# JeffWang987/MVSTER

Measured on AMD Instinct MI355X. Metric: depth-maps/sec (DTU 512×640, 5-view, 4-stage) at 1/2/4/8 MI355X, higher is better.
Workload: dtype f32; 1 GPU; DTU mid 512x640, 5 views, 4-stage cascade 8/8/4/4 hyp, B=1 eval, 1 depth map(s) per step per GPU; launch=hipGraph replay, parallelism=replicas x1, depth_maps_in_flight_per_gpu=2

## Files before the change

### include/mvster_hip.h

```cpp
#ifndef MVSTER_HIP_H
#define MVSTER_HIP_H

#ifdef __cplusplus
extern "C" {
#endif

#define MVSTER_OK 0
#define MVSTER_ERR_NULL (-1)
#define MVSTER_ERR_SHAPE (-2)
#define MVSTER_ERR_UNSUPPORTED (-3)
#define MVSTER_ERR_LAUNCH (-4)

int mvster_relative_projection(const float* proj_matrices, float* rt, int B, int N, void* stream);

int mvster_relative_projection_multi(const float* const* proj_matrices, int nstage, float* rt, int B, int N,
                                     void* stream);

int mvster_pack_images(const float* const* imgs, int N, float* out, int B, int H, int W, void* stream);

int mvster_pack_images_u8(const unsigned char* imgs, float* out, int V, int H, int W, void* stream);

int mvster_load_pack_images_u8(const unsigned char* buf, long buf_bytes, const int* desc_host, const int* desc, const void* tables,
                               long table_words, float* out, unsigned char* out_u8, int V, int Hd, int Wd, void* stream);

// ... 36 lines not shown
                                long* origin_ints);

int mvster_warp_agg_bwd_sorted_scratch(int B, int NV, int C, int D, int h, int w, int Hs, int Ws, long* rec_floats, long* ints);
int mvster_warp_agg_bwd_sorted(const float* ref_feat, const float* src_feat, const float* rt, const float* hypo,
                               const float* out, const float* wsum, const float* grad_out, float* grad_ref, float* grad_src,
                               float* rec, int* ints, int B, int NV, int C, int G, int D, int h, int w, int Hs, int Ws,
                               long ref_batch_stride, long src_view_stride, long src_batch_stride, int group_cor,
                               int attn_fuse_d, float attn_temp, void* stream);

int mvster_init_range(const float* depth_values, int ndv, float* out, int B, int D, int h, int w, int inverse,
                      void* stream);

int mvster_schedule_inverse_range(const float* inv_min, const float* inv_max, float* out, int B, int D, int h,
                                  int w, void* stream);

int mvster_schedule_range(const float* cur_depth, const float* interval, float* out, int B, int D, int h, int w,
                          void* stream);

int mvster_select_depth(const float* logits, const float* feat, const float* prob_w, const float* prob_b, int CF,
                        const float* hypo, float* attn, float* depth, float* conf, float* inv_min, float* inv_max,
                        float* logits_out, int B, int D, int h, int w, float split_itv, void* stream);

int mvster_select_depth_bwd(const float* attn, const float* gattn, const float* feat, const float* prob_w, float* dfeat,
                            float* partial, int B, int D, int h, int w, int CF, void* stream);

int mvster_upsample_bilinear(const float* in, float* out, int B, int hi, int wi, int ho, int wo, void* stream);

int mvster_upsample_bilinear_multi(const float* const* ins, float* const* outs, const int* his, const int* wis, int n, int B,
                                   int ho, int wo, void* stream);

int mvster_conv_mfma(const float* in, const float* wpk, const float* scale, const float* shift, const float* skip,
                     const float* zeros, const float* prob_w, const float* prob_b, float* out, const int* geom,
                     int ngeom, const long* woff, int cin, int mt, int nt, int variant, void* stream);

int mvster_conv_small(const float* in, const float* w, const float* scale, const float* shift, const float* skip,
                      float* out, int NB, int H, int W, int cin, int relu, void* stream);

int mvster_conv_narrow(const float* in, const float* w, const float* scale, const float* shift, const float* skip,
                       float* out, int NB, int H, int W, int cin, int relu, int mt, int wpc, void* stream);

int mvster_conv_narrow4(const float* in, const float* w, const float* scale, const float* shift, float* out, int NB, int H,
                        int W, int relu, int mt, int wpc, void* stream);

int mvster_conv_narrow_pair(const float* in, const float* w1, const float* scale1, const float* shift1, const float* w2,
                            const float* scale2, const float* shift2, float* out, int NB, int H, int W, int relu1, int relu2,
                            int wpc, void* stream);

int mvster_conv_narrow_pair_planes(const float* const* imgs, int N, int B, int H, int W, const float* w1, const float* scale1,
                                   const float* shift1, const float* w2, const float* scale2, const float* shift2, float* out,
                                   int relu1, int relu2, int wpc, const float* const* proj_matrices, int nstage, float* rt,
                                   const float* depth_values, int ndv, float* hypo, int D, int h, int w, int inverse,
                                   void* stream);

int mvster_deconv_small(const float* in, const float* w, const float* scale, const float* shift, const float* skip,
                        const float* prob_w, const float* prob_b, float* out, int NB, int Hi, int Wi, int cin,
                        int cout, int relu, void* stream);

int mvster_deconv_select(const float* in, const float* w, const float* scale, const float* shift, const float* skip,
                         const float* prob_w, const float* prob_b, const float* hypo, float* attn, float* depth, float* conf,
                         float* inv_min, float* inv_max, float* logits_out, int B, int D, int Hi, int Wi, int cin, int relu,
                         float split_itv, void* stream);

int mvster_deconv_select_riders(const float* in, const float* w, const float* scale, const float* shift, const float* skip,
                                const float* prob_w, const float* prob_b, const float* hypo, float* attn, float* depth,
                                float* conf, float* inv_min, float* inv_max, float* logits_out, int B, int D, int Hi, int Wi,
                                int cin, int relu, float split_itv, const float* const* up_ins, float* const* up_outs,
// ... 199 lines not shown
```

### mvster_amd/_lib.py

```python
import ctypes
import os

_HERE = os.path.dirname(os.path.abspath(__file__))
LIB_PATH = os.environ.get("MVSTER_LIB") or os.path.join(_HERE, "csrc", "libmvster_hip.so")

ERR_NULL, ERR_SHAPE, ERR_UNSUPPORTED, ERR_LAUNCH = -1, -2, -3, -4
ERRORS = {-1: "NULL pointer", -2: "bad shape", -3: "unsupported channel/tile combination", -4: "kernel launch failed"}

_f = ctypes.c_void_p
_i = ctypes.c_int
_l = ctypes.c_long
_fl = ctypes.c_float

SIGNATURES = {
    "mvster_relative_projection": [_f, _f, _i, _i, _f],
    "mvster_relative_projection_multi": [_f, _i, _f, _i, _i, _f],
    "mvster_pack_images": [_f, _i, _f, _i, _i, _i, _f],
    "mvster_pack_images_u8": [_f, _f, _i, _i, _i, _f],
    "mvster_load_pack_images_u8": [_f, _l, _f, _f, _f, _l, _f, _f, _i, _i, _i, _f],
    "mvster_forward_prologue": [_f, _i, _f, _i, _i, _i, _f, _i, _f, _f, _i, _f, _i, _i, _i, _i, _f],
    "mvster_warp_agg_fwd": [_f, _f, _f, _f, _f, _f] + [_i] * 9 + [_l] * 3 + [_i, _i, _fl, _i, _f],
    "mvster_warp_agg_fwd_indexed": [_f, _f, _f, _f, _f, _f] + [_i] * 10 + [_fl, _i, _f],
    "mvster_warp_agg_fwd_counted": [_f, _f, _f, _f, _f, _f] + [_i] * 9 + [_l] * 3 + [_i, _i, _fl, _i, _f, _f],
    "mvster_warp_agg_fwd_indexed_counted": [_f, _f, _f, _f, _f, _f] + [_i] * 10 + [_fl, _i, _f, _f],
    "mvster_gather_views": [_f, _f, _f, _i, _i, _i, _l, _f],
    "mvster_warp_agg_fwd_sched": [_f] * 6 + [_i, _f, _f, _f] + [_i] * 9 + [_l] * 3 + [_i, _fl, _i, _f],
    "mvster_warp_agg_bwd": [_f] * 11 + [_i] * 9 + [_l] * 3 + [_i, _i, _fl, _f],
    "mvster_warp_agg_bwd_scratch": [_i] * 8 + [_f, _f],
    "mvster_warp_agg_bwd_sorted_scratch": [_i] * 8 + [_f, _f],
    "mvster_warp_agg_bwd_sorted": [_f] * 11 + [_i] * 9 + [_l] * 3 + [_i, _i, _fl, _f],
    "mvster_init_range": [_f, _i, _f, _i, _i, _i, _i, _i, _f],
    "mvster_schedule_inverse_range": [_f, _f, _f, _i, _i, _i, _i, _f],
    "mvster_schedule_range": [_f, _f, _f, _i, _i, _i, _i, _f],
    "mvster_select_depth": [_f, _f, _f, _f, _i, _f, _f, _f, _f, _f, _f, _f, _i, _i, _i, _i, _fl, _f],
    "mvster_select_depth_bwd": [_f, _f, _f, _f, _f, _f, _i, _i, _i, _i, _i, _f],
    "mvster_upsample_bilinear": [_f, _f, _i, _i, _i, _i, _i, _f],
    "mvster_upsample_bilinear_multi": [_f, _f, _f, _f, _i, _i, _i, _i, _f],
    "mvster_conv_mfma": [_f, _f, _f, _f, _f, _f, _f, _f, _f, _f, _i, _f, _i, _i, _i, _i, _f],
    "mvster_conv_small": [_f, _f, _f, _f, _f, _f, _i, _i, _i, _i, _i, _f],
    "mvster_conv_narrow": [_f, _f, _f, _f, _f, _f, _i, _i, _i, _i, _i, _i, _i, _f],
    "mvster_conv_narrow4": [_f, _f, _f, _f, _f, _i, _i, _i, _i, _i, _i, _f],
    "mvster_conv_narrow_pair": [_f, _f, _f, _f, _f, _f, _f, _f, _i, _i, _i, _i, _i, _i, _f],
    "mvster_conv_narrow_pair_planes": [_f] + [_i] * 4 + [_f] * 7 + [_i] * 3 + [_f, _i, _f, _f, _i, _f] + [_i] * 4 + [_f],
    "mvster_deconv_select": [_f] * 14 + [_i] * 6 + [_fl, _f],
    "mvster_deconv_select_riders": [_f] * 14 + [_i] * 6 + [_fl] + [_f] * 4 + [_i] * 3 + [_f],
    "mvster_deconv_small": [_f, _f, _f, _f, _f, _f, _f, _f, _i, _i, _i, _i, _i, _i, _f],
    "mvster_fpn_tail_gather": [_f, _f, _f, _f, _i, _i, _i, _i, _f],
    "mvster_fpn_lateral_up": [_f, _f, _f, _f, _f, _i, _i, _i, _i, _i, _f],
    "mvster_fpn_tail_fused": [_f, _f, _f, _f, _f, _f, _i, _i, _i, _i, _f],
    "mvster_fpn_tail_gather_bwd": [_f, _f, _i, _i, _i, _i, _i, _f],
    "mvster_pack_conv_weights": [_f, _f] + [_i] * 6 + [_l] * 5 + [_i, _f],
    "mvster_pack_wino_weights": [_f, _f, _i, _i, _i, _i, _l, _l, _l, _l, _l, _i, _f],
    "mvster_pack_wino_batch": [_f, _i, _i, _f],
    "mvster_pack_conv_weights_classes": [_f, _f, _i, _i, _i, _i, _i, _f, _f, _f, _f],
    "mvster_conv_wgrad": [_f, _f, _f] + [_i] * 20 + [_f],
    "mvster_conv_wgrad_slots": [_i] * 12,
    "mvster_bn_relu_fwd": [_f, _f, _f, _f, _f, _l, _i, _i, _i, _f],
    "mvster_conv_wgrad_finish": [_f, _f] + [_i] * 10 + [_f],
    "mvster_bn_slots": [_l, _i, _i],
    "mvster_col_sum": [_f, _f, _f, _f, _l, _i, _f],
    "mvster_bn_train_slots": [_l, _i, _i],
    "mvster_bn_train_fwd": [_f] * 10 + [_l, _i, _i, _i, _fl, _fl, _f],
    "mvster_bn_train_bwd": [_f] * 7 + [_l, _i, _i, _i, _f],
    "mvster_conv_wgrad_finish_batch": [_f, _i, _f],
    "mvster_bn_relu_bwd_reduce": [_f] * 11 + [_l, _i, _i, _i, _f],
    "mvster_bn_relu_bwd_apply": [_f] * 8 + [_l, _i, _i, _i, _i, _f],
    "mvster_upsample2x_cl_fwd": [_f, _f, _i, _i, _i, _i, _f],
    "mvster_upsample2x_cl_bwd": [_f, _f, _i, _i, _i, _i, _f],
    "mvster_upsample2x_nearest_cl": [_f, _f, _i, _i, _i, _i, _i, _f],
    "mvster_sinkhorn": [_f, _f, _f, _f, _f, _i, _i, _l, _i, _fl, _f],
    "mvster_sinkhorn_continuous": [_f, _f, _f, _f, _f, _f, _i, _i, _l, _i, _fl, _f],
# ... 83 lines not shown
```

### mvster_amd/conv_plan.py

```python
import ctypes

import numpy as np
import torch

from . import _lib, ops

GEOM = ("B", "Di", "Hi", "Wi", "Do", "Ho", "Wo", "DoF", "HoF", "WoF", "sd", "sh", "sw", "cout", "ntile_total", "relu",
        "skip_mode", "osd", "osh", "osw", "nclass")
GEOM_CLASS = ("kd", "kh", "kw", "pd", "ph", "pw", "od", "oh", "ow", "nsteps")

SKIP_NONE, SKIP_ADD, SKIP_UPSAMPLE_ADD = 0, 1, 2


def _pack_gemm(wk):
    K, N = wk.shape
    Kp, Np = (K + 15) // 16 * 16, (N + 15) // 16 * 16
    full = wk.new_zeros(Kp, Np)
    full[:K, :N] = wk
    return full.view(Kp // 16, 4, 4, Np // 16, 16).permute(0, 3, 1, 4, 2).contiguous().view(-1), Kp // 16


def fold_bn(bn, cout, device):
    if bn is None:
        return torch.ones(cout, device=device), torch.zeros(cout, device=device)
# ... 68 lines not shown


FUSE_TAIL = True
FUSE_SELECT = True
LDS_BUDGET = 12 * 256 * 16
FORCE_VARIANT = None
TPERS16_MIN_VOXELS = 40960
FUSE_CONV0 = True
NARROW_PAIR_WPC = 1
NARROW_PAIR_MIN_PIXELS = 512 * 14 * 64
NARROW_MIN_VOXELS = 64 * 256


def _lds_plan(B, Do, Ho, Wo, kernel, stride, ntile_total):
    kd, kh, kw = kernel
    if kw not in (3, 5) or Wo < 24:
        return None
    for mt in (4, 2):
        ty = 2 * mt
        patch = kd * ((ty - 1) * stride[1] + kh) * (31 * stride[2] + kw) * 64
        if patch > LDS_BUDGET or (mt == 4 and Ho < 6):
            continue
        blocks = -(-Wo // 32) * -(-Ho // ty) * Do * B
        nt = max(n for n in (4, 2, 1) if n <= ntile_total and ntile_total % n == 0)
        while nt > 1 and blocks * (ntile_total // nt) < 512:
            nt //= 2
        return mt, nt
    return None


WINO_RING_INSTANCES = {(0, 1, 3), (0, 2, 3), (1, 2, 3), (2, 2, 3), (0, 4, 3), (1, 4, 3), (2, 4, 3),
                       (0, 4, 1), (1, 4, 1), (2, 4, 1), (0, 2, 1), (1, 2, 1), (2, 2, 1), (0, 1, 1), (2, 1, 1)}
WINO_INSTANCES = {(1, 1), (2, 1), (2, 2), (1, 2)}


def _wino_plan(layer, B, Do, Ho, Wo):
    tiles = B * Do * -(-Ho // 8) * -(-Wo // 32)
    kd = layer.kernel[0]
    if kd == 1 and layer.cin in (16, 32):
        nt = 2 if layer.ntile_total % 2 == 0 else 1
        if tiles * (layer.ntile_total // nt) >= 192:
            return 8 | (1 << 8), 2, nt
        return None
    nt = 2 if (layer.ntile_total % 2 == 0 and tiles * (layer.ntile_total // 2) >= 224) else 1
    if (1, layer.cin // 16, kd) not in WINO_RING_INSTANCES:
        nt = 1
    if tiles * (layer.ntile_total // nt) >= 160 and (0 if nt == 1 else 1, layer.cin // 16, kd) in WINO_RING_INSTANCES:
        return 9, 2, nt
    return None


def _tiles(M, ntile_total, nclass):
    best = None
    for nt in (5, 4, 3, 2, 1):
        if nt > ntile_total or ntile_total % nt:
            continue
        for mt in (4, 2, 1):
            waves = -(-M // (16 * mt)) * (ntile_total // nt) * nclass
            if waves >= 2048:
                return mt, nt
            if best is None or waves > best[0]:
                best = (waves, mt, nt)
    return best[1], best[2]


class ConvLayer:
# ... 182 lines not shown
            ntaps = np.zeros(len(self.classes), dtype=np.int32)
            taps = np.zeros((len(self.classes), 27), dtype=np.int32)
            for i, c in enumerate(self.classes):
                kzs, kys, kxs = c["taps"]
                flat = [(z * kh + y) * kw + x for z in kzs for y in kys for x in kxs]
                ntaps[i] = len(flat)
                taps[i, :len(flat)] = flat
            tab = self._class_pack = (ntaps, np.ascontiguousarray(self.woff, dtype=np.int64), taps)
        ntaps, woff, taps = tab
        rc = _lib.load().mvster_pack_conv_weights_classes(
            w.data_ptr(), self.wpk.data_ptr(), self.cout, self._cin_raw, self.cin, kd * kh * kw, len(self.classes),
            ntaps.ctypes.data_as(ctypes.c_void_p), woff.ctypes.data_as(ctypes.c_void_p), taps.ctypes.data_as(ctypes.c_void_p),
            ops._stream())
        _lib.check(rc, "pack_conv_weights_classes")
        if self.w_deconv is not None:
            self.w_deconv.copy_(w[:, :, 0].permute(2, 3, 0, 1))

    def repack(self, weight, bias=None):
        w = weight.detach().float()
        if w.dim() == 4:
            w = w.unsqueeze(2)
        self._pack(w)
        if bias is not None:
            self.shift[:self.cout] = bias.detach().float() * self.scale[:self.cout]

    def out_shape(self, B, Di, Hi, Wi):
        kd, kh, kw = self.kernel
        s, p = self.stride, self.padding
        if self.transposed:
            return (B, Di * s[0], Hi * s[1], Wi * s[2])
        return (B, (Di + 2 * p[0] - kd) // s[0] + 1, (Hi + 2 * p[1] - kh) // s[1] + 1, (Wi + 2 * p[2] - kw) // s[2] + 1)

    def _geom(self, B, Di, Hi, Wi, skip_mode):
        key = (B, Di, Hi, Wi, skip_mode)
        g = self._geom_cache.get(key)
        if g is None:
            _, DoF, HoF, WoF = self.out_shape(B, Di, Hi, Wi)
            s = self.stride
            if self.transposed:
                Do, Ho, Wo = Di, Hi, Wi
                sd = sh = sw = 1
                osd, osh, osw = s
            else:
                Do, Ho, Wo = DoF, HoF, WoF
                sd, sh, sw = s
                osd = osh = osw = 1
            vals = dict(B=B, Di=Di, Hi=Hi, Wi=Wi, Do=Do, Ho=Ho, Wo=Wo, DoF=DoF, HoF=HoF, WoF=WoF, sd=sd, sh=sh, sw=sw,
                        cout=self.cout, ntile_total=self.ntile_total, relu=int(self.relu), skip_mode=skip_mode,
                        osd=osd, osh=osh, osw=osw, nclass=len(self.classes))
            arr = [vals[k] for k in GEOM]
            for c in self.classes:
                arr += [c[k] for k in GEOM_CLASS]
            mt, nt = _tiles(B * Do * Ho * Wo, self.ntile_total, len(self.classes))
            variant = 0
            lds = None
            if not self.transposed and self.cin % 16 == 0 and skip_mode in (SKIP_NONE, SKIP_ADD):
                lds = _lds_plan(B, Do, Ho, Wo, self.kernel, self.stride, self.ntile_total)
            if lds is not None and FORCE_VARIANT != 0:
                variant, (mt, nt) = 1, lds
            if variant == 0 and self.cin >= 16 and FORCE_VARIANT is None:
                tiles16 = -(-(B * Do * Ho * Wo) // 16)
                waves = -(-tiles16 // mt) * (self.ntile_total // nt) * len(self.classes)
                if waves < 1024 and min(c["nsteps"] for c in self.classes) >= 8:
                    variant, mt = 2, 1
                    nt = 1
                    for cand in (4, 2):
                        if self.ntile_total % cand == 0 and tiles16 * (self.ntile_total // cand) * len(self.classes) >= 512:
                            nt = cand
                            break
            if (FORCE_VARIANT is None and self.wpk_wino is not None and self.prob is None
                    and skip_mode in (SKIP_NONE, SKIP_ADD)):
                wv = _wino_plan(self, B, Do, Ho, Wo)
                if wv is not None:
                    variant, mt, nt = wv
            tuned = tuned_choice(self, B, Di, Hi, Wi, skip_mode)[0] if FORCE_VARIANT is None else None
            if tuned and (tuned[0] & 0xff) in (8, 9) and (self.wpk_wino is None or self.prob is not None):
                tuned = None
            if tuned:
                variant, mt, nt = tuned
            if self.w_small is not None and skip_mode in (SKIP_NONE, SKIP_ADD) and FORCE_VARIANT in (None, 3, 10):
                if FORCE_VARIANT is not None:
                    variant, mt, nt = FORCE_VARIANT, 0, 0
                elif tuned and tuned[0] in (3, 10):
                    variant, mt, nt = tuned
                else:
                    variant, mt, nt = (10, 0, 0) if B * Do * Ho * Wo >= NARROW_MIN_VOXELS else (3, 0, 0)
                if variant == 10 and not hasattr(_lib.load(), "mvster_conv_narrow"):
                    variant = 3
            if (getattr(self, "w_small4", None) is not None and skip_mode == SKIP_NONE and FORCE_VARIANT is None
                    and self.prob is None and B * Do * Ho * Wo >= NARROW_MIN_VOXELS and hasattr(_lib.load(), "mvster_conv_narrow4")):
                variant, mt, nt = 10, 0, 0
            if self.w_deconv is not None and skip_mode in (SKIP_NONE, SKIP_ADD) and FORCE_VARIANT in (None, 4):
                variant = 4
                if (FORCE_VARIANT is None and self.prob is None and self.cin == 16 and self.cout == 8
                        and B * Di * Hi * Wi >= TPERS16_MIN_VOXELS):
                    variant, mt, nt = 5, 2, 1
            if (FORCE_VARIANT is None and self.transposed and self.kernel == (1, 5, 5) and self.stride == (1, 2, 2)
                    and self.padding == (0, 2, 2) and self.cin in (16, 32) and self.prob is None
                    and skip_mode in (SKIP_NONE, SKIP_ADD) and B * Di * Hi * Wi >= TPERS16_MIN_VOXELS):
                variant, mt, nt = 5, 2, 1
            g = (np.asarray(arr, dtype=np.int32), mt, nt, (B, DoF, HoF, WoF), variant)
            self._geom_cache[key] = g
        return g

    def __call__(self, x, skip=None, skip_mode=SKIP_NONE, tiles=None):
        B, Di, Hi, Wi, C = x.shape
        if C != self.cin or not x.is_contiguous() or x.dtype != torch.float32 or not x.is_cuda:
            raise RuntimeError("conv_mfma: bad input (shape %s, cin %d)" % (tuple(x.shape), self.cin))
        if skip is None:
            skip_mode = SKIP_NONE
        geom, mt, nt, oshape, variant = self._geom(B, Di, Hi, Wi, skip_mode)
        if tiles is not None:
# ... 394 lines not shown
```

### mvster_amd/csrc/conv_mfma.hip

```cpp
#include <stdlib.h>

#include <type_traits>

#include "conv_args.hpp"

namespace {

using namespace mvconv;

typedef unsigned u32x4v __attribute__((ext_vector_type(4)));

#ifdef MVSTER_TIMELINE
__device__ unsigned long long* g_tl = nullptr;
#define MV_TL(k)                                                                                              \
    do {                                                                                                      \
        __builtin_amdgcn_sched_barrier(0);                                                                    \
        if (g_tl && (threadIdx.x & 63) == 0)                                                                  \
            g_tl[((size_t)blockIdx.x * 4 + (threadIdx.x >> 6)) * 8 + (k)] = __builtin_amdgcn_s_memtime();     \
        __builtin_amdgcn_sched_barrier(0);                                                                    \
    } while (0)
#define MV_TL_ID()                                                                                            \
    do {                                                                                                      \
        if (g_tl && (threadIdx.x & 63) == 0) {                                                                \
            g_tl[((size_t)blockIdx.x * 4 + (threadIdx.x >> 6)) * 8 + 6] = __builtin_amdgcn_s_getreg(63492);   \
// ... 34 lines not shown
            for (int j = 0; j < 4; ++j) v[j] += k[j];
        } else if (a.skip_mode == 2) {
            const int hh = a.HoF / 2, wh = a.WoF / 2;
            const mv::Lerp ly = mv::make_lerp(oy, hh, a.HoF), lx = mv::make_lerp(ox, wh, a.WoF);
            const float* sk = a.skip + (long)b * hh * wh * a.cout + n0;
            const f32x4v k00 = *reinterpret_cast<const f32x4v*>(sk + ((long)ly.i0 * wh + lx.i0) * a.cout);
            const f32x4v k01 = *reinterpret_cast<const f32x4v*>(sk + ((long)ly.i0 * wh + lx.i1) * a.cout);
            const f32x4v k10 = *reinterpret_cast<const f32x4v*>(sk + ((long)ly.i1 * wh + lx.i0) * a.cout);
            const f32x4v k11 = *reinterpret_cast<const f32x4v*>(sk + ((long)ly.i1 * wh + lx.i1) * a.cout);
#pragma unroll
            for (int j = 0; j < 4; ++j) v[j] = mv::bilerp(ly, lx, k00[j], k01[j], k10[j], k11[j]) + v[j];
        }
        *reinterpret_cast<f32x4v*>(op) = v;
    } else {
        for (int j = 0; j < 4; ++j) {
            if (n0 + j >= a.cout) break;
            float r = v[j];
            if (a.skip_mode == 1) r += a.skip[opix * a.cout + n0 + j];
            op[j] = r;
        }
    }
}

__device__ __forceinline__ void epilogue_store(const ConvArgs& a, f32x4v v, int n0, long opix, int b, int oy, int ox) {
    epilogue_store(a, v, n0, opix, b, oy, ox, *reinterpret_cast<const f32x4v*>(a.scale + n0),
                   *reinterpret_cast<const f32x4v*>(a.shift + n0));
}

constexpr int conv_min_waves(int mt, int nt) {
    const int t = mt * nt;
    return t <= 2 ? 5 : (t <= 4 ? 4 : (t <= 8 ? 3 : 2));
}

template <int CIN, int MT, int NT, bool SPLITK>
__global__ void __launch_bounds__(256, conv_min_waves(MT, NT)) conv_mfma_kernel(ConvArgs a) {
    static_assert(CIN % 4 == 0 && (CIN >= 16 ? CIN % 16 == 0 : 16 % CIN == 0), "channel packing");
    __shared__ f32x4v red[SPLITK ? 3 * MT * NT * 64 : 1];

    const int cls = blockIdx.z;
    const int KD = a.kd[cls], KH = a.kh[cls], KW = a.kw[cls];
    const int PD = a.pd[cls], PH = a.ph[cls], PW = a.pw[cls];
    const int ntaps = KD * KH * KW;
    const mvtaps::TapDivs tdv = a.tapdiv[cls];
    const int nsteps_all = a.nsteps[cls];
    const bool no_pad = a.all_inside[cls] != 0;
    const bool fit = mvtaps::masks_fit(KD, KH, KW);

    const int lane = threadIdx.x & 63;
    const int wave = __builtin_amdgcn_readfirstlane(threadIdx.x >> 6);
    const int lm = lane & 15;
    const int lq = lane >> 4;
    const unsigned Mtot = (unsigned)(a.B * a.Do * a.Ho * a.Wo);
    const int nt0 = blockIdx.y * NT;
    const unsigned ntiles = (Mtot + 15u) >> 4;
    const unsigned ngroups = SPLITK ? (ntiles + MT - 1) / MT : (ntiles + 4 * MT - 1) / (4 * MT);
    for (unsigned grp0 = blockIdx.x; grp0 < ngroups; grp0 += gridDim.x) {
    const unsigned grp = gridDim.x == ngroups ? xcd_remap(grp0, ngroups) : grp0;
    const unsigned tile0 = SPLITK ? grp * MT : (grp * 4u + wave) * MT;
    if (!SPLITK && tile0 * 16u >= Mtot) break;

    int iz0[MT], iy0[MT], ix0[MT];
    unsigned abase[MT];
    unsigned vmask[MT];
    int opix[MT];
    int oyx[MT];
#pragma unroll
    for (int mt = 0; mt < MT; ++mt) {
        unsigned m = (tile0 + mt) * 16u + lm;
        const bool ok = m < Mtot;
        if (!ok) m = 0;
        unsigned r = fast_div(m, a.Wo, a.div_mul[0], a.div_shr[0]);
        const int x = (int)(m - r * (unsigned)a.Wo);
        unsigned r2 = fast_div(r, a.Ho, a.div_mul[1], a.div_shr[1]);
        const int y = (int)(r - r2 * (unsigned)a.Ho);
        const unsigned b = fast_div(r2, a.Do, a.div_mul[2], a.div_shr[2]);
        const int z = (int)(r2 - b * (unsigned)a.Do);
        iz0[mt] = ok ? z * a.sd - PD : -(1 << 20);
        iy0[mt] = y * a.sh - PH;
        ix0[mt] = x * a.sw - PW;
        const int pin0 = (((int)b * a.Di + (ok ? iz0[mt] : 0)) * a.Hi + iy0[mt]) * a.Wi + ix0[mt];
        abase[mt] = (unsigned)(pin0 * CIN + (CIN >= 16 ? lq * 4 : 0)) * 4u;
        vmask[mt] = fit ? mvtaps::voxel_mask(iz0[mt], iy0[mt], ix0[mt], KD, KH, KW, a.Di, a.Hi, a.Wi) : 0u;
        const int oz = z * a.osd + a.od[cls], oy = y * a.osh + a.oh[cls], ox = x * a.osw + a.ow[cls];
        opix[mt] = ok ? (((int)b * a.DoF + oz) * a.HoF + oy) * a.WoF + ox : -1;
        oyx[mt] = (oy << 16) | ox;
    }

    f32x4v acc[MT][NT];
#pragma unroll
    for (int mt = 0; mt < MT; ++mt)
#pragma unroll
        for (int nt = 0; nt < NT; ++nt) acc[mt][nt] = (f32x4v){0.f, 0.f, 0.f, 0.f};

    const long wstep = (long)a.ntile_total * 1024;
    const __amdgpu_buffer_rsrc_t w_rsrc = __builtin_amdgcn_make_buffer_rsrc(
        const_cast<float*>(a.wpk + a.woff[cls] + (long)nt0 * 256), (short)0,
        (int)((unsigned)nsteps_all * (unsigned)wstep - (unsigned)nt0 * 1024u), 0x00020000);
    const unsigned wlane = (unsigned)lane * 16u;

    const __amdgpu_buffer_rsrc_t in_rsrc =
        __builtin_amdgcn_make_buffer_rsrc(const_cast<float*>(a.in), (short)0, (int)a.in_bytes, 0x00020000);
    const int nsteps = mvtaps::wave_steps(nsteps_all, wave, SPLITK);

    auto uni = [](unsigned v) { return CIN >= 16 ? (unsigned)__builtin_amdgcn_readfirstlane((int)v) : v; };
    auto load_step = [&](auto mode, int si, f32x4v (&A)[MT], f32x4v (&Bv)[NT]) {
        constexpr int MODE = decltype(mode)::value;
        const int s = mvtaps::wave_step(si, wave, SPLITK);
        const int tap = mvtaps::step_tap<CIN>(s, lq);
        const int c = CIN >= 16 ? s * 16 - tap * CIN : mvtaps::step_channel<CIN>(s, lq);
        const bool tap_ok = CIN >= 16 || tap < ntaps;
        const mvtaps::Tap t = mvtaps::tap_decode(tap_ok ? tap : 0, KH, KW, tdv);
        const unsigned uoff = uni((unsigned)(mvtaps::tap_offset(t, a.Hi, a.Wi) * CIN + c) * 4u);
        const unsigned sel = MODE == 1 ? uni(mvtaps::tap_select(t, KD, KH)) : 0u;
#pragma unroll
        for (int mt = 0; mt < MT; ++mt) {
            if constexpr (MODE == 0) {
                A[mt] = __builtin_bit_cast(f32x4v, __builtin_amdgcn_raw_buffer_load_b128(in_rsrc, abase[mt], uoff, 0));
            } else {
                const bool ok = tap_ok && (MODE == 1 ? mvtaps::tap_inside(vmask[mt], sel)
                                                     : mvtaps::tap_inside_cmp(iz0[mt], iy0[mt], ix0[mt], t, a.Di, a.Hi, a.Wi));
                const unsigned off = ok ? abase[mt] + uoff : 0xFFFFFFF0u;
                A[mt] = __builtin_bit_cast(f32x4v, __builtin_amdgcn_raw_buffer_load_b128(in_rsrc, off, 0, 0));
            }
        }
        const unsigned woff = (unsigned)s * (unsigned)wstep;
#pragma unroll
        for (int nt = 0; nt < NT; ++nt)
            Bv[nt] = __builtin_bit_cast(f32x4v, __builtin_amdgcn_raw_buffer_load_b128(w_rsrc, wlane + nt * 1024u, woff, 0));
    };

    auto mma_step = [&](const f32x4v (&A)[MT], const f32x4v (&Bv)[NT]) {
#pragma unroll
        for (int j = 0; j < 4; ++j)
#pragma unroll
            for (int mt = 0; mt < MT; ++mt)
#pragma unroll
                for (int nt = 0; nt < NT; ++nt)
                    acc[mt][nt] = __builtin_amdgcn_mfma_f32_16x16x4f32(Bv[nt][j], A[mt][j], acc[mt][nt], 0, 0, 0);
    };

    auto k_loop = [&](auto mode) {
        f32x4v af[MT], bf[NT], ag[MT], bg[NT];
        if (nsteps <= 0) return;
        const int last = nsteps - 1;
        load_step(mode, 0, af, bf);
        int s = 0;
        for (; s + 2 <= nsteps; s += 2) {
            load_step(mode, s + 1, ag, bg);
            mma_step(af, bf);
            load_step(mode, min(s + 2, last), af, bf);
            mma_step(ag, bg);
        }
        if (s < nsteps) mma_step(af, bf);
    };
    if (!fit) {
        f32x4v af[MT], bf[NT];
        for (int s = 0; s < nsteps; ++s) {
            load_step(std::integral_constant<int, 2>{}, s, af, bf);
            mma_step(af, bf);
        }
    } else if (CIN >= 16 && no_pad) {
        k_loop(std::integral_constant<int, CIN >= 16 ? 0 : 1>{});
    } else {
        k_loop(std::integral_constant<int, 1>{});
    }

    if (SPLITK) {
        if (wave > 0) {
#pragma unroll
            for (int mt = 0; mt < MT; ++mt)
#pragma unroll
                for (int nt = 0; nt < NT; ++nt) red[((wave - 1) * MT * NT + mt * NT + nt) * 64 + lane] = acc[mt][nt];
        }
        __syncthreads();
        if (wave > 0) return;
#pragma unroll
        for (int w = 0; w < 3; ++w)
#pragma unroll
            for (int mt = 0; mt < MT; ++mt)
#pragma unroll
                for (int nt = 0; nt < NT; ++nt) {
                    const f32x4v r = red[(w * MT * NT + mt * NT + nt) * 64 + lane];
#pragma unroll
                    for (int j = 0; j < 4; ++j) acc[mt][nt][j] += r[j];
                }
    }

#pragma unroll
    for (int mt = 0; mt < MT; ++mt) {
        if (opix[mt] < 0) continue;
        const int b = a.skip_mode == 2 ? opix[mt] / (a.DoF * a.HoF * a.WoF) : 0;
#pragma unroll
        for (int nt = 0; nt < NT; ++nt) {
            const int n0 = (nt0 + nt) * 16 + lq * 4;
            if (n0 >= a.cout) continue;
            epilogue_store(a, acc[mt][nt], n0, opix[mt], b, oyx[mt] >> 16, oyx[mt] & 0xffff);
        }
    }
    }
}

template <int CIN, int MT, int NT, bool SPLITK>
int launch(const ConvArgs& a, hipStream_t s) {
    const long Mtot = (long)a.B * a.Do * a.Ho * a.Wo;
    if (Mtot >= (1L << 31) || (long)a.B * a.Di * a.Hi * a.Wi >= (1L << 31)) return MVSTER_ERR_SHAPE;
    const long tiles = (Mtot + 15) / 16;
    const long per_block = SPLITK ? MT : 4 * MT;
    long gx = (tiles + per_block - 1) / per_block;
    dim3 grid((unsigned)gx, a.ntile_total / NT, a.nclass);
    MV_NOTE_KERNEL("conv_mfma_kernel<%d, %d, %d, %s>", CIN, MT, NT, SPLITK ? "true" : "false");
    hipLaunchKernelGGL((conv_mfma_kernel<CIN, MT, NT, SPLITK>), grid, dim3(256), 0, s, a);
    return mv_check_launch();
}

template <int CIN>
int dispatch_tiles(const ConvArgs& a, int MT, int NT, bool splitk, hipStream_t s) {
    if (splitk) {
        if constexpr (CIN >= 16) {
#define MV_S(M_, N_) if (MT == M_ && NT == N_) return launch<CIN, M_, N_, true>(a, s);
            MV_S(1, 1) MV_S(1, 2) MV_S(1, 4) MV_S(2, 1) MV_S(2, 2)
#undef MV_S
        }
        return MVSTER_ERR_UNSUPPORTED;
    }
#define MV_T(M_, N_) if (MT == M_ && NT == N_) return launch<CIN, M_, N_, false>(a, s);
    MV_T(1, 1) MV_T(2, 1) MV_T(4, 1) MV_T(1, 2) MV_T(2, 2) MV_T(4, 2) MV_T(1, 4) MV_T(2, 4) MV_T(4, 4)
    if constexpr (CIN == 64) {
        MV_T(1, 5) MV_T(2, 5) MV_T(4, 5)
        MV_T(1, 3) MV_T(2, 3) MV_T(4, 3) MV_T(1, 9) MV_T(2, 9)
    }
#undef MV_T
    return MVSTER_ERR_UNSUPPORTED;
}

struct LdsDivs {
    unsigned mul[6], shr[6];
};
constexpr int kMaxStage = 12;
__device__ __forceinline__ int patch_plane(int npix) { return ((npix * 2 + 7) & ~7) + 4; }
static const bool g_no_wlds = MV_PROBE_ENV("MVSTER_NO_WLDS") != nullptr;

template <int MT, int NT, int KW, int NG, int WN>
__global__ void __launch_bounds__(256) conv_lds_kernel(ConvArgs a, int tiles_x, int tiles_y, LdsDivs dv) {
    extern __shared__ __attribute__((aligned(16))) float patch_raw[];
    MV_TL(0);
    MV_TL_ID();
    f32x4v* patch_base = reinterpret_cast<f32x4v*>(patch_raw);
    f32x4v* wl = patch_base + NG * 1024 + 32;
    constexpr int TY = 2 * MT;
// ... 251 lines not shown
        if (a.kd[c] * a.kh[c] * a.kw[c] > kMaxTaps || a.nsteps[c] < 1) return MVSTER_ERR_SHAPE;
        if (a.kd[c] < 1 || a.kh[c] < 1 || a.kw[c] < 1) return MVSTER_ERR_SHAPE;
        a.tapdiv[c] = mvtaps::make_tap_divs(a.kh[c], a.kw[c]);
    }
    if (a.B <= 0 || a.Do <= 0 || a.Ho <= 0 || a.Wo <= 0 || a.cout <= 0 || a.ntile_total <= 0) return MVSTER_ERR_SHAPE;
    find_divisor((unsigned)a.Wo, a.div_mul[0], a.div_shr[0]);
    find_divisor((unsigned)a.Ho, a.div_mul[1], a.div_shr[1]);
    find_divisor((unsigned)a.Do, a.div_mul[2], a.div_shr[2]);
    {
        const long in_elems = (long)a.B * a.Di * a.Hi * a.Wi * cin;
        const long out_elems = (long)a.B * a.DoF * a.HoF * a.WoF * a.cout;
        if (in_elems >= (1L << 30) || out_elems >= (1L << 31)) return MVSTER_ERR_SHAPE;
        a.in_bytes = (unsigned)(in_elems * 4);
    }
    for (int c = 0; c < a.nclass; ++c) {
        auto inside = [](int n_out, int s, int p, int k, int extent) {
            return -p >= 0 && (n_out - 1) * s - p + (k - 1) < extent;
        };
        a.all_inside[c] = inside(a.Do, a.sd, a.pd[c], a.kd[c], a.Di) && inside(a.Ho, a.sh, a.ph[c], a.kh[c], a.Hi) &&
                          inside(a.Wo, a.sw, a.pw[c], a.kw[c], a.Wi);
    }
    if (a.skip_mode != 0 && !skip) return MVSTER_ERR_NULL;
    if (a.ntile_total % nt != 0) return MVSTER_ERR_SHAPE;
    hipStream_t s = (hipStream_t)stream;
    a.cin = cin;
    if ((variant & 0xff) == 5) return dispatch_pers(a, mt, nt, variant >> 8, s);
    if ((variant & 0xff) == 6) return dispatch_1x1(a, mt, variant >> 8, s);
    if ((variant & 0xff) == 7) return dispatch_pp(a, mt, nt, s);
    if ((variant & 0xff) == 8) return dispatch_wino(a, nt, variant >> 8, false, s);
    if ((variant & 0xff) == 9) return dispatch_wino(a, nt, variant >> 8, true, s);
    if ((variant & 0xff) == 11) return dispatch_b3(a, mt, variant >> 8, s);
    if (prob_w && (a.cout != 8 || a.skip_mode == 2 || variant == 1)) return MVSTER_ERR_UNSUPPORTED;
    if (variant == 1) return dispatch_lds(a, mt, nt, s);
    if (variant != 0 && variant != 2) return MVSTER_ERR_UNSUPPORTED;
    const bool splitk = variant == 2;
    switch (cin) {
        case 4: return dispatch_tiles<4>(a, mt, nt, splitk, s);
        case 8: return dispatch_tiles<8>(a, mt, nt, splitk, s);
        case 16: return dispatch_tiles<16>(a, mt, nt, splitk, s);
        case 32: return dispatch_tiles<32>(a, mt, nt, splitk, s);
        case 64: return dispatch_tiles<64>(a, mt, nt, splitk, s);
        case 80: return dispatch_tiles<80>(a, mt, nt, splitk, s);
        default: return MVSTER_ERR_UNSUPPORTED;
    }
}

#ifdef MVSTER_TIMELINE
extern "C" int mvster_debug_timeline(void* buf) {
    return hipMemcpyToSymbol(HIP_SYMBOL(g_tl), &buf, sizeof(buf)) == hipSuccess ? MVSTER_OK : MVSTER_ERR_LAUNCH;
}
#endif

extern "C" int mvster_mfma_probe(const float* A, const float* B, float* D, void* stream) {
    if (!A || !B || !D) return MVSTER_ERR_NULL;
    hipLaunchKernelGGL(mfma_probe_kernel, dim3(1), dim3(64), 0, (hipStream_t)stream, A, B, D);
    return mv_check_launch();
}

namespace {
__global__ void __launch_bounds__(256) pack_weights_kernel(const float* __restrict__ w, float* __restrict__ wpk, int nsteps,
                                                           int ntile, int cout, int cin, int cin_pad, int kd, int kh, int kw,
                                                           long s_n, long s_c, long s_z, long s_y, long s_x, int flip) {
    const int idx = blockIdx.x * 256 + threadIdx.x;
    if (idx >= nsteps * ntile * 64) return;
    const int lane = idx & 63, t = (idx >> 6) % ntile, st = (idx >> 6) / ntile;
    const int n = t * 16 + (lane & 15);
    const int ntaps = kd * kh * kw;
    f32x4v out;
#pragma unroll
    for (int j = 0; j < 4; ++j) {
        const int k = st * 16 + (lane >> 4) * 4 + j;
        const int tap = k / cin_pad, ci = k - tap * cin_pad;
        float v = 0.0f;
        if (tap < ntaps && ci < cin && n < cout) {
            int kx = tap % kw, ky = (tap / kw) % kh, kz = tap / (kw * kh);
            if (flip) { kx = kw - 1 - kx; ky = kh - 1 - ky; kz = kd - 1 - kz; }
            v = w[(long)n * s_n + (long)ci * s_c + (long)kz * s_z + (long)ky * s_y + (long)kx * s_x];
// ... 72 lines not shown
```

### mvster_amd/csrc/conv_taps.h

```cpp
#pragma once

#if defined(__HIPCC__)
#define MVT_HD __host__ __device__ __forceinline__
#else
#define MVT_HD inline
#endif

namespace mvtaps {

struct TapDivs {
    unsigned kw_mul, kw_shr, kw_one, kh_mul, kh_shr, kh_one;
};

struct Tap {
    int kz, ky, kx;
};

MVT_HD unsigned mulhi(unsigned a, unsigned b) { return (unsigned)(((unsigned long long)a * b) >> 32); }

MVT_HD unsigned div_ms(unsigned n, unsigned mul, unsigned shr, unsigned one) { return (mulhi(n, mul) >> shr) | (n & one); }

inline void make_tap_div(int d, unsigned& mul, unsigned& shr, unsigned& one) {
    mul = 0u; shr = 0u; one = ~0u;
    if (d <= 1) return;
// ... 26 lines not shown
    Tap t;
    t.kx = tap - (int)r * KW;
    t.ky = (int)r - (int)z * KH;
    t.kz = (int)z;
    return t;
}

MVT_HD int tap_offset(const Tap& t, int Hi, int Wi) { return (t.kz * Hi + t.ky) * Wi + t.kx; }

MVT_HD bool masks_fit(int KD, int KH, int KW) { return KD + KH + KW <= 32; }

MVT_HD unsigned axis_mask(int i0, int K, int extent) {
    const int lo = i0 < 0 ? -i0 : 0;
    const int hi = extent - i0 < K ? extent - i0 : K;
    if (hi <= lo) return 0u;
    return ((1u << hi) - 1u) & ~((1u << lo) - 1u);
}

MVT_HD unsigned voxel_mask(int iz0, int iy0, int ix0, int KD, int KH, int KW, int Di, int Hi, int Wi) {
    return axis_mask(iz0, KD, Di) | (axis_mask(iy0, KH, Hi) << KD) | (axis_mask(ix0, KW, Wi) << (KD + KH));
}

MVT_HD unsigned tap_select(const Tap& t, int KD, int KH) {
    return (1u << t.kz) | (1u << (KD + t.ky)) | (1u << (KD + KH + t.kx));
}

MVT_HD bool tap_inside(unsigned vmask, unsigned sel) { return (vmask & sel) == sel; }

MVT_HD bool tap_inside_cmp(int iz0, int iy0, int ix0, const Tap& t, int Di, int Hi, int Wi) {
    return (unsigned)(iz0 + t.kz) < (unsigned)Di && (unsigned)(iy0 + t.ky) < (unsigned)Hi &&
           (unsigned)(ix0 + t.kx) < (unsigned)Wi;
}

MVT_HD int wave_steps(int nsteps_all, int wave, bool splitk) { return splitk ? (nsteps_all - wave + 3) / 4 : nsteps_all; }
MVT_HD int wave_step(int si, int wave, bool splitk) { return splitk ? wave + 4 * si : si; }

}
```

### mvster_amd/graph.py

```python
import collections

import torch


def _sample_layout(imgs, proj_matrices, depth_values):
    segs, off = [], 0
    for name, t in ([("img%d" % i, t) for i, t in enumerate(imgs)] + [("proj_" + k, proj_matrices[k]) for k in sorted(proj_matrices)]
                    + [("depth_values", depth_values)]):
        segs.append((name, off, tuple(t.shape)))
        off += (t.numel() + 63) // 64 * 64
    return segs, off


def pack_sample(imgs, proj_matrices, depth_values, pin=True):
    segs, total = _sample_layout(imgs, proj_matrices, depth_values)
    flat = torch.zeros(total, dtype=torch.float32)
    if pin:
        flat = flat.pin_memory()
    src = {("img%d" % i): t for i, t in enumerate(imgs)}
    src.update({"proj_" + k: v for k, v in proj_matrices.items()})
    src["depth_values"] = depth_values
    for name, off, shape in segs:
        flat[off:off + src[name].numel()].copy_(src[name].reshape(-1).float().cpu())
    return flat
# ... 105 lines not shown
            else:
                yield (k,), v

    def load(self, imgs, proj_matrices, depth_values):
        src = list(imgs) + [proj_matrices[k] for k in self._proj_keys] + [depth_values]
        torch._foreach_copy_(self._dst, src)

    def replay(self):
        self.graph.replay()
        fresh = torch.empty(self._out_total, dtype=torch.float32, device=self.flat.device)
        new = [fresh.as_strided(shape, stride, off) for _, off, shape, stride in self._slots]
        torch._foreach_copy_(new, self._src)
        out = {}
        for path, j in self._paths:
            if len(path) == 1:
                out[path[0]] = new[j]
            else:
                out.setdefault(path[0], {})[path[1]] = new[j]
        return {k: out[k] for k in self.outputs}


class ForwardCache:

    def __init__(self, capacity=4):
        self.capacity = capacity
        self.entries = collections.OrderedDict()
        self.stats = {"eager": 0, "captured": 0, "replayed": 0, "capture_failed": 0}
        self.disabled_keys = set()

    @staticmethod
    def key(model, imgs, proj_matrices, depth_values):
        im = imgs[0]
        from . import conv_plan, ops
        glob = (conv_plan.FORCE_VARIANT, conv_plan.FUSE_TAIL, conv_plan.FUSE_CONV0, conv_plan.NARROW_PAIR_WPC, conv_plan.FUSE_SELECT, conv_plan.LDS_BUDGET, conv_plan.NARROW_MIN_VOXELS,
                id(conv_plan._TUNING), ops.WGRAD_MAX_SLOTS)
        cfg = (glob, model.warp_variant, getattr(model, "fuse_hypotheses", None), getattr(model, "merge_launches", None), model.overlap_streams, float(model.attn_temp), model.attn_fuse_d, model.num_stage,
               tuple(model.stage_splits), tuple(model.depth_interals_ratio), tuple(model.group_cor_dim))
        return (im.device.index, len(imgs), tuple(im.shape), int(depth_values.shape[1]), tuple(sorted(proj_matrices.keys())), cfg)

    def clear(self):
        self.entries.clear()

    def __call__(self, model, imgs, proj_matrices, depth_values):
        key = self.key(model, imgs, proj_matrices, depth_values)
        if key in self.disabled_keys:
            self.stats["eager"] += 1
            return model._forward_eval(imgs, proj_matrices, depth_values)
        stamp = model._state_stamp()
        hit = self.entries.get(key)
        if hit is not None and hit[0] == stamp:
            self.entries.move_to_end(key)
            if hit[1] is None:
                try:
                    hit[1] = _CachedForward(model, imgs, proj_matrices, depth_values)
                    self.stats["captured"] += 1
                except RuntimeError as e:
                    import warnings
                    warnings.warn("mvster_amd: hipGraph capture of the eval forward failed for %r (%s): this shape stays on "
                                  "eager launches" % (key, str(e)[:200]))
                    self.stats["capture_failed"] += 1
                    self.disabled_keys.add(key)
                    del self.entries[key]
                    return model._forward_eval(imgs, proj_matrices, depth_values)
            else:
                hit[1].load(imgs, proj_matrices, depth_values)
            self.stats["replayed"] += 1
            return hit[1].replay()
# ... 293 lines not shown
```

Before: 1180 depth-maps/s.

## Add 8/16-wave split-K MFMA conv kernels for small cost-volume layers

Generalizes the split-K MFMA 3D conv kernel so each block can use 8 or 16 waves instead of 4, all sharing the K reduction. Partial accumulators are reduced through LDS, and each of the first MT*NT waves finishes one output tile. The plan picks this variant for a hard-coded table of small-spatial layer signatures. The goal is more in-flight work per block on low-occupancy small layers, at the cost of extra LDS traffic, a barrier, and idle waves during the epilogue.

```diff
diff --git a/include/mvster_hip.h b/include/mvster_hip.h
--- a/include/mvster_hip.h
+++ b/include/mvster_hip.h
@@ -92,6 +92,8 @@
 int mvster_conv_mfma(const float* in, const float* wpk, const float* scale, const float* shift, const float* skip,
                      const float* zeros, const float* prob_w, const float* prob_b, float* out, const int* geom,
                      int ngeom, const long* woff, int cin, int mt, int nt, int variant, void* stream);
+
+int mvster_conv_splitk_waves(int cin, int mt, int nt, int kwaves);
 
 int mvster_conv_small(const float* in, const float* w, const float* scale, const float* shift, const float* skip,
                       float* out, int NB, int H, int W, int cin, int relu, void* stream);
diff --git a/mvster_amd/_lib.py b/mvster_amd/_lib.py
--- a/mvster_amd/_lib.py
+++ b/mvster_amd/_lib.py
@@ -37,6 +37,7 @@
     "mvster_upsample_bilinear": [_f, _f, _i, _i, _i, _i, _i, _f],
     "mvster_upsample_bilinear_multi": [_f, _f, _f, _f, _i, _i, _i, _i, _f],
     "mvster_conv_mfma": [_f, _f, _f, _f, _f, _f, _f, _f, _f, _f, _i, _f, _i, _i, _i, _i, _f],
+    "mvster_conv_splitk_waves": [_i, _i, _i, _i],
     "mvster_conv_small": [_f, _f, _f, _f, _f, _f, _i, _i, _i, _i, _i, _f],
     "mvster_conv_narrow": [_f, _f, _f, _f, _f, _f, _i, _i, _i, _i, _i, _i, _i, _f],
     "mvster_conv_narrow4": [_f, _f, _f, _f, _f, _i, _i, _i, _i, _i, _i, _f],
diff --git a/mvster_amd/conv_plan.py b/mvster_amd/conv_plan.py
--- a/mvster_amd/conv_plan.py
+++ b/mvster_amd/conv_plan.py
@@ -124,6 +124,29 @@
 WINO_RING_INSTANCES = {(0, 1, 3), (0, 2, 3), (1, 2, 3), (2, 2, 3), (0, 4, 3), (1, 4, 3), (2, 4, 3),
                        (0, 4, 1), (1, 4, 1), (2, 4, 1), (0, 2, 1), (1, 2, 1), (2, 2, 1), (0, 1, 1), (2, 1, 1)}
 WINO_INSTANCES = {(1, 1), (2, 1), (2, 2), (1, 2)}
+
+SPLITK_WAVE_INSTANCES = {(1, 1, 8), (1, 2, 8), (1, 4, 8), (2, 1, 8), (2, 2, 8), (2, 4, 8), (4, 2, 8),
+                         (1, 1, 16), (1, 2, 16), (1, 4, 16), (2, 1, 16), (2, 2, 16)}
+SPLITK_WAVE_CIN = (16, 32, 64)
+SPLITK_WAVES = True
+SPLITK_WAVE_LAYERS = {
+    "C32-32_k3x3x3_s1x1x1_1x8x16x20_sk0": (8, 1, 2),
+    "C32-32_k3x3x3_s1x1x1_1x8x32x40_sk0": (8, 1, 2),
+    "C64-64_k3x3x3_s1x1x1_1x8x16x20_sk0": (8, 1, 4),
+    "C16-32_k1x3x3_s1x2x2_1x8x32x40_sk0": (8, 1, 2),
+    "C32-64_k1x3x3_s1x2x2_1x8x32x40_sk0": (8, 1, 4),
+    "C32-64_k1x3x3_s1x2x2_1x4x128x160_sk0": (8, 1, 4),
+    "T64-32_k1x3x3_s1x2x2_1x8x16x20_sk1": (8, 1, 2),
+    "T64-32_k1x3x3_s1x2x2_1x4x32x40_sk1": (8, 2, 2),
+}
+
+
+def splitk_wave_choice(sig):
+    hit = SPLITK_WAVE_LAYERS.get(sig) if SPLITK_WAVES else None
+    if hit is None or not hasattr(_lib.load(), "mvster_conv_splitk_waves"):
+        return None
+    kwaves, mt, nt = hit
+    return 2 | (kwaves << 8), mt, nt
 
 
 def _wino_plan(layer, B, Do, Ho, Wo):
@@ -372,7 +395,7 @@
         return (B, (Di + 2 * p[0] - kd) // s[0] + 1, (Hi + 2 * p[1] - kh) // s[1] + 1, (Wi + 2 * p[2] - kw) // s[2] + 1)
 
     def _geom(self, B, Di, Hi, Wi, skip_mode):
-        key = (B, Di, Hi, Wi, skip_mode)
+        key = (B, Di, Hi, Wi, skip_mode, SPLITK_WAVES)
         g = self._geom_cache.get(key)
         if g is None:
             _, DoF, HoF, WoF = self.out_shape(B, Di, Hi, Wi)
@@ -418,6 +441,10 @@
                 tuned = None
             if tuned:
                 variant, mt, nt = tuned
+            if variant == 2 and FORCE_VARIANT is None:
+                wide = splitk_wave_choice(layer_signature(self, B, Di, Hi, Wi, skip_mode))
+                if wide is not None:
+                    variant, mt, nt = wide
             if self.w_small is not None and skip_mode in (SKIP_NONE, SKIP_ADD) and FORCE_VARIANT in (None, 3, 10):
                 if FORCE_VARIANT is not None:
                     variant, mt, nt = FORCE_VARIANT, 0, 0
diff --git a/mvster_amd/csrc/conv_mfma.hip b/mvster_amd/csrc/conv_mfma.hip
--- a/mvster_amd/csrc/conv_mfma.hip
+++ b/mvster_amd/csrc/conv_mfma.hip
@@ -90,10 +90,16 @@
     return t <= 2 ? 5 : (t <= 4 ? 4 : (t <= 8 ? 3 : 2));
 }
 
-template <int CIN, int MT, int NT, bool SPLITK>
-__global__ void __launch_bounds__(256, conv_min_waves(MT, NT)) conv_mfma_kernel(ConvArgs a) {
+constexpr int conv_red_slabs(int mt, int nt, bool splitk, int kwaves) {
+    return !splitk ? 0 : (kwaves == 4 ? 3 * mt * nt : kwaves * mt * nt - 1);
+}
+
+template <int CIN, int MT, int NT, bool SPLITK, int KWAVES = 4>
+__global__ void __launch_bounds__(64 * KWAVES, KWAVES == 4 ? conv_min_waves(MT, NT) : 4) conv_mfma_kernel(ConvArgs a) {
     static_assert(CIN % 4 == 0 && (CIN >= 16 ? CIN % 16 == 0 : 16 % CIN == 0), "channel packing");
-    __shared__ f32x4v red[SPLITK ? 3 * MT * NT * 64 : 1];
+    static_assert(KWAVES == 4 || (SPLITK && (KWAVES == 8 || KWAVES == 16)), "K waves");
+    static_assert(conv_red_slabs(MT, NT, SPLITK, KWAVES) <= 64, "static LDS");
+    __shared__ f32x4v red[SPLITK ? conv_red_slabs(MT, NT, SPLITK, KWAVES) * 64 : 1];
 
     const int cls = blockIdx.z;
     const int KD = a.kd[cls], KH = a.kh[cls], KW = a.kw[cls];
@@ -158,12 +164,12 @@
 
     const __amdgpu_buffer_rsrc_t in_rsrc =
         __builtin_amdgcn_make_buffer_rsrc(const_cast<float*>(a.in), (short)0, (int)a.in_bytes, 0x00020000);
-    const int nsteps = mvtaps::wave_steps(nsteps_all, wave, SPLITK);
+    const int nsteps = mvtaps::wave_steps(nsteps_all, wave, SPLITK, KWAVES);
 
     auto uni = [](unsigned v) { return CIN >= 16 ? (unsigned)__builtin_amdgcn_readfirstlane((int)v) : v; };
     auto load_step = [&](auto mode, int si, f32x4v (&A)[MT], f32x4v (&Bv)[NT]) {
         constexpr int MODE = decltype(mode)::value;
-        const int s = mvtaps::wave_step(si, wave, SPLITK);
+        const int s = mvtaps::wave_step(si, wave, SPLITK, KWAVES);
         const int tap = mvtaps::step_tap<CIN>(s, lq);
         const int c = CIN >= 16 ? s * 16 - tap * CIN : mvtaps::step_channel<CIN>(s, lq);
         const bool tap_ok = CIN >= 16 || tap < ntaps;
@@ -223,7 +229,37 @@
         k_loop(std::integral_constant<int, 1>{});
     }
 
-    if (SPLITK) {
+    if constexpr (SPLITK && KWAVES != 4) {
+        constexpr int T = MT * NT;
+#pragma unroll
+        for (int mt = 0; mt < MT; ++mt)
+#pragma unroll
+            for (int nt = 0; nt < NT; ++nt) {
+                const int t = mt * NT + nt;
+                if (t > 0 || wave > 0) red[(wave * T + t - 1) * 64 + lane] = acc[mt][nt];
+            }
+        __syncthreads();
+        if (wave >= T) return;
+        f32x4v v = acc[0][0];
+        if (wave > 0) v = red[(wave - 1) * 64 + lane];
+#pragma unroll
+        for (int w = 1; w < KWAVES; ++w) {
+            const f32x4v r = red[(w * T + wave - 1) * 64 + lane];
+#pragma unroll
+            for (int j = 0; j < 4; ++j) v[j] += r[j];
+        }
+        const int mtd = wave / NT, ntd = wave - mtd * NT;
+        int op = opix[0], yx = oyx[0];
+#pragma unroll
+        for (int mt = 1; mt < MT; ++mt)
+            if (mtd == mt) { op = opix[mt]; yx = oyx[mt]; }
+        const int n0 = (nt0 + ntd) * 16 + lq * 4;
+        if (op >= 0 && n0 < a.cout) {
+            const int b = a.skip_mode == 2 ? op / (a.DoF * a.HoF * a.WoF) : 0;
+            epilogue_store(a, v, n0, op, b, yx >> 16, yx & 0xffff);
+        }
+        return;
+    } else if (SPLITK) {
         if (wave > 0) {
 #pragma unroll
             for (int mt = 0; mt < MT; ++mt)
@@ -258,7 +294,7 @@
     }
 }
 
-template <int CIN, int MT, int NT, bool SPLITK>
+template <int CIN, int MT, int NT, bool SPLITK, int KWAVES = 4>
 int launch(const ConvArgs& a, hipStream_t s) {
     const long Mtot = (long)a.B * a.Do * a.Ho * a.Wo;
     if (Mtot >= (1L << 31) || (long)a.B * a.Di * a.Hi * a.Wi >= (1L << 31)) return MVSTER_ERR_SHAPE;
@@ -266,13 +302,27 @@
     const long per_block = SPLITK ? MT : 4 * MT;
     long gx = (tiles + per_block - 1) / per_block;
     dim3 grid((unsigned)gx, a.ntile_total / NT, a.nclass);
-    MV_NOTE_KERNEL("conv_mfma_kernel<%d, %d, %d, %s>", CIN, MT, NT, SPLITK ? "true" : "false");
-    hipLaunchKernelGGL((conv_mfma_kernel<CIN, MT, NT, SPLITK>), grid, dim3(256), 0, s, a);
+    if constexpr (KWAVES == 4) MV_NOTE_KERNEL("conv_mfma_kernel<%d, %d, %d, %s>", CIN, MT, NT, SPLITK ? "true" : "false");
+    else MV_NOTE_KERNEL("conv_mfma_kernel<%d, %d, %d, true, %d>", CIN, MT, NT, KWAVES);
+    hipLaunchKernelGGL((conv_mfma_kernel<CIN, MT, NT, SPLITK, KWAVES>), grid, dim3(64 * KWAVES), 0, s, a);
     return mv_check_launch();
 }
 
+#define MV_SPLITK_WAVE_TILES(X)                                                          \
+    X(1, 1, 8) X(1, 2, 8) X(1, 4, 8) X(2, 1, 8) X(2, 2, 8) X(2, 4, 8) X(4, 2, 8)         \
+    X(1, 1, 16) X(1, 2, 16) X(1, 4, 16) X(2, 1, 16) X(2, 2, 16)
+constexpr bool splitk_wave_cin(int cin) { return cin == 16 || cin == 32 || cin == 64; }
+
 template <int CIN>
-int dispatch_tiles(const ConvArgs& a, int MT, int NT, bool splitk, hipStream_t s) {
+int dispatch_tiles(const ConvArgs& a, int MT, int NT, bool splitk, int kwaves, hipStream_t s) {
+    if (splitk && kwaves != 4) {
+        if constexpr (splitk_wave_cin(CIN)) {
+#define MV_SK(M_, N_, K_) if (MT == M_ && NT == N_ && kwaves == K_) return launch<CIN, M_, N_, true, K_>(a, s);
+            MV_SPLITK_WAVE_TILES(MV_SK)
+#undef MV_SK
+        }
+        return MVSTER_ERR_UNSUPPORTED;
+    }
     if (splitk) {
         if constexpr (CIN >= 16) {
 #define MV_S(M_, N_) if (MT == M_ && NT == N_) return launch<CIN, M_, N_, true>(a, s);
@@ -590,17 +640,26 @@
     if ((variant & 0xff) == 11) return dispatch_b3(a, mt, variant >> 8, s);
     if (prob_w && (a.cout != 8 || a.skip_mode == 2 || variant == 1)) return MVSTER_ERR_UNSUPPORTED;
     if (variant == 1) return dispatch_lds(a, mt, nt, s);
-    if (variant != 0 && variant != 2) return MVSTER_ERR_UNSUPPORTED;
-    const bool splitk = variant == 2;
+    const int kwaves = (variant & 0xff) == 2 && (variant >> 8) != 0 ? variant >> 8 : 4;
+    if (variant != 0 && variant != 2 && !((variant & 0xff) == 2 && (kwaves == 8 || kwaves == 16))) return MVSTER_ERR_UNSUPPORTED;
+    const bool splitk = (variant & 0xff) == 2;
     switch (cin) {
-        case 4: return dispatch_tiles<4>(a, mt, nt, splitk, s);
-        case 8: return dispatch_tiles<8>(a, mt, nt, splitk, s);
-        case 16: return dispatch_tiles<16>(a, mt, nt, splitk, s);
-        case 32: return dispatch_tiles<32>(a, mt, nt, splitk, s);
-        case 64: return dispatch_tiles<64>(a, mt, nt, splitk, s);
-        case 80: return dispatch_tiles<80>(a, mt, nt, splitk, s);
+        case 4: return dispatch_tiles<4>(a, mt, nt, splitk, kwaves, s);
+        case 8: return dispatch_tiles<8>(a, mt, nt, splitk, kwaves, s);
+        case 16: return dispatch_tiles<16>(a, mt, nt, splitk, kwaves, s);
+        case 32: return dispatch_tiles<32>(a, mt, nt, splitk, kwaves, s);
+        case 64: return dispatch_tiles<64>(a, mt, nt, splitk, kwaves, s);
+        case 80: return dispatch_tiles<80>(a, mt, nt, splitk, kwaves, s);
         default: return MVSTER_ERR_UNSUPPORTED;
     }
+}
+
+extern "C" int mvster_conv_splitk_waves(int cin, int mt, int nt, int kwaves) {
+    if (!splitk_wave_cin(cin)) return 0;
+#define MV_SK(M_, N_, K_) if (mt == M_ && nt == N_ && kwaves == K_) return 1;
+    MV_SPLITK_WAVE_TILES(MV_SK)
+#undef MV_SK
+    return 0;
 }
 
 #ifdef MVSTER_TIMELINE
diff --git a/mvster_amd/csrc/conv_taps.h b/mvster_amd/csrc/conv_taps.h
--- a/mvster_amd/csrc/conv_taps.h
+++ b/mvster_amd/csrc/conv_taps.h
@@ -82,7 +82,11 @@
            (unsigned)(ix0 + t.kx) < (unsigned)Wi;
 }
 
-MVT_HD int wave_steps(int nsteps_all, int wave, bool splitk) { return splitk ? (nsteps_all - wave + 3) / 4 : nsteps_all; }
-MVT_HD int wave_step(int si, int wave, bool splitk) { return splitk ? wave + 4 * si : si; }
+MVT_HD int wave_steps(int nsteps_all, int wave, bool splitk, int kwaves = 4) {
+    return splitk ? (kwaves == 4 ? (nsteps_all - wave + 3) / 4 : (nsteps_all - wave + kwaves - 1) / kwaves) : nsteps_all;
+}
+MVT_HD int wave_step(int si, int wave, bool splitk, int kwaves = 4) {
+    return splitk ? (kwaves == 4 ? wave + 4 * si : wave + kwaves * si) : si;
+}
 
 }
diff --git a/mvster_amd/graph.py b/mvster_amd/graph.py
--- a/mvster_amd/graph.py
+++ b/mvster_amd/graph.py
@@ -161,7 +161,7 @@
     def key(model, imgs, proj_matrices, depth_values):
         im = imgs[0]
         from . import conv_plan, ops
-        glob = (conv_plan.FORCE_VARIANT, conv_plan.FUSE_TAIL, conv_plan.FUSE_CONV0, conv_plan.NARROW_PAIR_WPC, conv_plan.FUSE_SELECT, conv_plan.LDS_BUDGET, conv_plan.NARROW_MIN_VOXELS,
+        glob = (conv_plan.FORCE_VARIANT, conv_plan.SPLITK_WAVES, conv_plan.FUSE_TAIL, conv_plan.FUSE_CONV0, conv_plan.NARROW_PAIR_WPC, conv_plan.FUSE_SELECT, conv_plan.LDS_BUDGET, conv_plan.NARROW_MIN_VOXELS,
                 id(conv_plan._TUNING), ops.WGRAD_MAX_SLOTS)
         cfg = (glob, model.warp_variant, getattr(model, "fuse_hypotheses", None), getattr(model, "merge_launches", None), model.overlap_streams, float(model.attn_temp), model.attn_fuse_d, model.num_stage,
                tuple(model.stage_splits), tuple(model.depth_interals_ratio), tuple(model.group_cor_dim))
```

After: 1183 depth-maps/s, median of 6. Within noise of the previous version (+0.2%).
